# mokemokechicken/reversi-alpha-zero

Hardware: NVIDIA H100
Metric: self_play_games_per_sec (higher is better)
Workload: dtype f16

## Files before the change

### reversi-alpha-zero_b200/csrc/rz_net_tc.cu

```cuda
#include <stdlib.h>
#include <mutex>
#include <type_traits>
#include "rz_bitboard.cuh"
#include "rz_net.cuh"
#include "rz_tc_common.cuh"

namespace rz {
namespace tc {

constexpr int kThreads = 384;
constexpr uint32_t kProducerRegs = 40, kMathRegs = 232;
constexpr int kMathThreads = 256;
constexpr uint32_t kActCg = 2896, kActSlot = 144;
constexpr uint32_t kActBytes = 32 * kActCg;
constexpr uint32_t kStageBytes = 32768, kStages = 3;
constexpr int kResAhead = 4;
constexpr uint32_t kA0Bytes = 8192, kW0Bytes = 16384;
constexpr uint32_t kOffAct = 0;
constexpr uint32_t kOffW = kOffAct + kActBytes;
constexpr uint32_t kOffA0 = kOffW + kStages * kStageBytes;
constexpr uint32_t kOffW0 = kOffA0 + kA0Bytes;
constexpr uint32_t kOffSS = kOffW0 + kW0Bytes;
constexpr uint32_t kOffHw = kOffSS + 2 * 2048;
constexpr uint32_t kOffBar = kOffHw + 768 * 4;
constexpr uint32_t kNumBars = 2 * kStages + 1;
constexpr uint32_t kSmemBytes = kOffBar + kNumBars * 8;
constexpr uint32_t kSmemAlloc = kSmemBytes + 128;
static_assert(kSmemAlloc <= 232448, "shared memory budget exceeded");
static_assert(kTowerResFloatsPerCta == (size_t)kMathThreads * 128, "residual scratch per CTA");

#ifdef RZ_TOWER_STAMPS
enum : int {
    kStTiles,
    kStTile,
    kStKLoop,
    kStFull,
    kStMma,
    kStEpiBar,
    kStEpi0,
    kStEpi1,
    kStEpi2,
    kStEpiLast,
    kStFeat,
    kStEmpty,
    kStCount
};
constexpr int kStMaxCtas = 1024;
__device__ unsigned long long g_tower_stamps[kStMaxCtas][kStCount];
__device__ __forceinline__ void stamp_add(int phase, uint32_t cycles) { atomicAdd(&g_tower_stamps[blockIdx.x][phase], (unsigned long long)cycles); }
#define RZ_STAMP(...) __VA_ARGS__
#else
#define RZ_STAMP(...)
#endif

template <int CL>
__global__ void __launch_bounds__(kThreads, 1) net_tower_kernel(const Params pp) {
    Params p = pp;
    if (p.n_dev) p.n = *p.n_dev;
    extern __shared__ uint8_t smem_raw[];
    const uint32_t base = (smem_u32(smem_raw) + 127u) & ~127u;
    uint8_t* sm = smem_raw + (base - smem_u32(smem_raw));
    const int warp = threadIdx.x >> 5, lane = threadIdx.x & 31;
    const uint32_t bar0 = base + kOffBar;
    auto bar_full = [&](uint32_t s) { return bar0 + s * 8; };
    auto bar_empty = [&](uint32_t s) { return bar0 + (kStages + s) * 8; };
    const uint32_t bar_w0 = bar0 + 2 * kStages * 8;
    const uint32_t ntiles = (p.n + 1) >> 1;
    const int L = p.n_layers;
    const uint32_t crank = CL > 1 ? cluster_ctarank() : 0u;
    const uint32_t cbase = blockIdx.x - crank;
    const uint32_t iters = cbase < ntiles ? (ntiles - cbase + gridDim.x - 1) / gridDim.x : 0u;

    for (uint32_t i = threadIdx.x * 16; i < kActBytes; i += kThreads * 16) *reinterpret_cast<uint4*>(sm + kOffAct + i) = make_uint4(0, 0, 0, 0);
    fence_proxy_async();
    for (uint32_t i = threadIdx.x; i < 768; i += kThreads)
        reinterpret_cast<float*>(sm + kOffHw)[i] = __ldg(i < 512 ? p.blob + p.off_policy_conv + i : p.blob + p.off_value_conv + (i - 512));
    if (threadIdx.x == 0) {
        for (uint32_t s = 0; s < kStages; ++s) { mbar_init(bar_full(s), 1); mbar_init(bar_empty(s), 8 * CL); }
        mbar_init(bar_w0, 1);
        asm volatile("fence.mbarrier_init.release.cluster;" ::: "memory");
    }
    __syncthreads();
    if (CL > 1) cluster_sync_all();

    if (warp >= 8) {
        asm volatile("setmaxnreg.dec.sync.aligned.u32 %0;" ::"n"(kProducerRegs));
        if (warp == 8 && lane == 0) {
            if (iters > 0) {
                mbar_expect_tx(bar_w0, kW0Bytes);
                bulk_g2s(base + kOffW0, p.w0, kW0Bytes, bar_w0);
            }
            uint32_t stage = 0, phase = 0;
            for (uint32_t it = 0; it < iters; ++it) {
                for (int l = 1; l < L; ++l) {
                    const uint8_t* src = reinterpret_cast<const uint8_t*>(p.w) + (size_t)(l - 1) * 36 * kStageBytes;
                    RZ_STAMP(uint32_t st_empty = 0;)
                    for (int s = 0; s < 36; ++s) {
                        RZ_STAMP(const uint32_t c0 = (uint32_t)clock();)
                        mbar_wait(bar_empty(stage), phase ^ 1);
                        RZ_STAMP(st_empty += (uint32_t)clock() - c0;)
                        mbar_expect_tx(bar_full(stage), kStageBytes);
                        if (CL == 1) {
                            bulk_g2s(base + kOffW + stage * kStageBytes, src + (size_t)s * kStageBytes, kStageBytes, bar_full(stage));
                        } else {
                            constexpr uint32_t kSlice = kStageBytes / CL;
                            bulk_g2s_mc(base + kOffW + stage * kStageBytes + crank * kSlice, src + (size_t)s * kStageBytes + crank * kSlice,
                                        kSlice, bar_full(stage), (uint16_t)((1u << CL) - 1u));
                        }
                        if (++stage == kStages) { stage = 0; phase ^= 1; }
                    }
                    RZ_STAMP(stamp_add(kStEmpty, st_empty);)
                }
            }
        }
    } else {
        asm volatile("setmaxnreg.inc.sync.aligned.u32 %0;" ::"n"(kMathRegs));
        const int et = threadIdx.x;
        const int wg = warp >> 2;
        const int r0 = wg * 64 + (warp & 3) * 16 + (lane >> 2);
        const int g0 = r0 >> 3, x = r0 & 7, y = g0 >> 1;
        const int cq = 2 * (lane & 3);
        const uint32_t act_row0 = base + kOffAct + (g0 + 2) * kActSlot + (x + 1) * 16 + cq * 2;
        const uint32_t act_row1 = act_row0 + kActSlot;
        const uint32_t a_wg = base + kOffAct + wg * 8 * kActSlot;
        float* ss_s = reinterpret_cast<float*>(sm + kOffSS);
        float4* res = reinterpret_cast<float4*>(p.res + (size_t)blockIdx.x * kTowerResFloatsPerCta) + et;
        const float* hw = reinterpret_cast<const float*>(sm + kOffHw);
        uint32_t stage = 0, phase = 0, ss_buf = 0;
        float d[128];
        ss_s[et] = __ldg(p.ss + et);
        ss_s[256 + et] = __ldg(p.ss + 256 + et);

        for (uint32_t it = 0; it < iters; ++it) {
            const uint32_t tile = blockIdx.x + it * gridDim.x;
            const uint32_t pos0 = tile * 2;
            RZ_STAMP(const uint32_t st_tile0 = (uint32_t)clock();)
            {
                const int m = et & 127, g = m >> 3, brd = g & 1;
                const bool valid = pos0 + brd < p.n;
                build_layer0_operand(sm + kOffA0, valid ? p.own[pos0 + brd] : 0, valid ? p.enemy[pos0 + brd] : 0, 2 * (et >> 7), g, m & 7,
                                     g >> 1);
                fence_proxy_async();
            }
            float hs[6];
            for (int l = 0; l < L; ++l) {
                const float* sc = ss_s + ss_buf * 512;
                const bool is_conv2 = l > 0 && (l & 1) == 0;
                float4 rb[kResAhead];
                RZ_STAMP(uint32_t st_c = (uint32_t)clock(), st_bar = 0, st_full = 0, st_mma = 0;)
                epi_bar();
                RZ_STAMP(st_bar += (uint32_t)clock() - st_c;)
                {
                    const size_t nl = l + 1 < L ? (size_t)l + 1 : 0;
                    const uint32_t dst = smem_u32(ss_s + (ss_buf ^ 1) * 512 + et);
                    cp_async_4(dst, p.ss + nl * 512 + et);
                    cp_async_4(dst + 1024, p.ss + nl * 512 + 256 + et);
                }
                RZ_STAMP(const uint32_t st_k0 = (uint32_t)clock();)
                acc_fence(d);
                if (l == 0) {
                    RZ_STAMP(st_c = (uint32_t)clock();)
                    mbar_wait(bar_w0, 0);
                    RZ_STAMP(st_full += (uint32_t)clock() - st_c;)
                    wgmma_fence();
#pragma unroll
                    for (uint32_t j = 0; j < 2; ++j)
                        wgmma_m64n256k16(d, smem_desc(base + kOffA0 + j * 2 * 2048 + wg * 1024, 2048, 128),
                                         smem_desc(base + kOffW0 + j * 2 * 4096, 4096, 128), j);
                    wgmma_commit();
                    RZ_STAMP(st_c = (uint32_t)clock();)
                    wgmma_wait<0>();
                    RZ_STAMP(st_mma += (uint32_t)clock() - st_c;)
                } else {
                    int prev = -1;
                    for (uint32_t tap = 0; tap < 9; ++tap) {
                        const uint32_t a_tap = a_wg + (2 * (tap / 3)) * kActSlot + (tap % 3) * 16;
                        for (uint32_t kb = 0; kb < 4; ++kb) {
                            RZ_STAMP(st_c = (uint32_t)clock();)
                            mbar_wait(bar_full(stage), phase);
                            RZ_STAMP(st_full += (uint32_t)clock() - st_c;)
                            const uint32_t b_st = base + kOffW + stage * kStageBytes;
                            wgmma_fence();
#pragma unroll
                            for (uint32_t j = 0; j < 4; ++j)
                                wgmma_m64n256k16(d, smem_desc(a_tap + (kb * 8 + 2 * j) * kActCg, kActCg, kActSlot),
                                                 smem_desc(b_st + 2 * j * 4096, 4096, 128), (tap | kb | j) != 0);
                            wgmma_commit();
                            RZ_STAMP(st_c = (uint32_t)clock();)
                            wgmma_wait<1>();
                            RZ_STAMP(st_mma += (uint32_t)clock() - st_c;)
                            if (prev >= 0 && lane == 0) {
                                mbar_arrive(bar_empty(prev));
                                if (CL > 1) mbar_arrive_cta(bar_empty(prev), crank ^ 1u);
                            }
                            prev = (int)stage;
                            if (++stage == kStages) { stage = 0; phase ^= 1; }
                        }
                    }
                    if (is_conv2) {
#pragma unroll
                        for (int i = 0; i < kResAhead; ++i) rb[i] = res[i * 256];
                    }
                    RZ_STAMP(st_c = (uint32_t)clock();)
                    wgmma_wait<0>();
                    RZ_STAMP(st_mma += (uint32_t)clock() - st_c;)
                    if (lane == 0) {
                        mbar_arrive(bar_empty(prev));
                        if (CL > 1) mbar_arrive_cta(bar_empty(prev), crank ^ 1u);
                    }
                }
                RZ_STAMP(const uint32_t st_k1 = (uint32_t)clock();)
                acc_fence(d);
                cp_async_wait_all();
                ss_buf ^= 1;
                const bool keep_res = l == 0 || is_conv2;
                const bool last = l == L - 1;
                RZ_STAMP(st_c = (uint32_t)clock();)
                if (!last) epi_bar();
                RZ_STAMP(const uint32_t st_e0 = (uint32_t)clock(); st_bar += st_e0 - st_c;)
                float* dbg0 = nullptr;
                float* dbg1 = nullptr;
                if (last && p.dbg_tower) {
                    if (pos0 < p.n) dbg0 = p.dbg_tower + ((size_t)pos0 * 64 + y * 8 + x) * 256;
                    if (pos0 + 1 < p.n) dbg1 = p.dbg_tower + ((size_t)(pos0 + 1) * 64 + y * 8 + x) * 256;
                }
                constexpr int kEpiRelu = 0, kEpiKeep = 1, kEpiLast = 2;
                auto epilogue = [&](auto conv2, auto kind) {
                    constexpr bool kConv2 = decltype(conv2)::value;
                    constexpr bool kKeep = decltype(kind)::value == kEpiKeep, kLast = decltype(kind)::value == kEpiLast;
                    if (kLast) {
#pragma unroll
                        for (int k = 0; k < 6; ++k) hs[k] = 0.f;
                    }
#pragma unroll
                for (int i = 0; i < 32; ++i) {
                    const int c = 8 * i + cq;
                    const float2 s = *reinterpret_cast<const float2*>(sc + c);
                    const float2 b = *reinterpret_cast<const float2*>(sc + 256 + c);
                    float v0 = fmaf(d[4 * i + 0], s.x, b.x), v1 = fmaf(d[4 * i + 1], s.y, b.y);
                    float v2 = fmaf(d[4 * i + 2], s.x, b.x), v3 = fmaf(d[4 * i + 3], s.y, b.y);
                    if (kConv2) {
                        const float4 r = rb[i % kResAhead];
                        if (i + kResAhead < 32) rb[i % kResAhead] = res[(i + kResAhead) * 256];
                        v0 += r.x; v1 += r.y; v2 += r.z; v3 += r.w;
                    }
                    if (kKeep || kLast) {
                        v0 = fmaxf(v0, 0.f); v1 = fmaxf(v1, 0.f); v2 = fmaxf(v2, 0.f); v3 = fmaxf(v3, 0.f);
                    }
                    if (!kLast) {
                        if (kKeep) res[i * 256] = make_float4(v0, v1, v2, v3);
                        const uint32_t h0 = pack_h2<!kKeep>(v0, v1);
                        const uint32_t h1 = pack_h2<!kKeep>(v2, v3);
                        const uint32_t off = (c >> 3) * kActCg;
                        asm volatile("st.shared.b32 [%0], %1;" ::"r"(act_row0 + off), "r"(h0) : "memory");
                        asm volatile("st.shared.b32 [%0], %1;" ::"r"(act_row1 + off), "r"(h1) : "memory");
                    } else {
                        const float4 w = *reinterpret_cast<const float4*>(hw + 2 * c);
                        const float2 wv = *reinterpret_cast<const float2*>(hw + 512 + c);
                        hs[0] = fmaf(v1, w.z, fmaf(v0, w.x, hs[0]));
                        hs[1] = fmaf(v1, w.w, fmaf(v0, w.y, hs[1]));
                        hs[2] = fmaf(v1, wv.y, fmaf(v0, wv.x, hs[2]));
                        hs[3] = fmaf(v3, w.z, fmaf(v2, w.x, hs[3]));
                        hs[4] = fmaf(v3, w.w, fmaf(v2, w.y, hs[4]));
                        hs[5] = fmaf(v3, wv.y, fmaf(v2, wv.x, hs[5]));
                        if (dbg0) *reinterpret_cast<float2*>(dbg0 + c) = make_float2(v0, v1);
                        if (dbg1) *reinterpret_cast<float2*>(dbg1 + c) = make_float2(v2, v3);
                    }
                }
                };
                using Conv2 = std::true_type;
                using NoConv2 = std::false_type;
                if (last) {
                    if (is_conv2) epilogue(Conv2(), std::integral_constant<int, kEpiLast>());
                    else epilogue(NoConv2(), std::integral_constant<int, kEpiLast>());
                } else if (is_conv2) {
                    epilogue(Conv2(), std::integral_constant<int, kEpiKeep>());
                } else if (keep_res) {
                    epilogue(NoConv2(), std::integral_constant<int, kEpiKeep>());
                } else {
                    epilogue(NoConv2(), std::integral_constant<int, kEpiRelu>());
                }
                if (!last) fence_proxy_async();
                RZ_STAMP(if (et == 0) {
                    stamp_add(kStKLoop, st_k1 - st_k0); stamp_add(kStFull, st_full); stamp_add(kStMma, st_mma); stamp_add(kStEpiBar, st_bar);
                    stamp_add(l == 0 ? kStEpi0 : last ? kStEpiLast : is_conv2 ? kStEpi2 : kStEpi1, (uint32_t)clock() - st_e0);
                })
            }
            RZ_STAMP(const uint32_t st_h0 = (uint32_t)clock();)
#pragma unroll
            for (int k = 0; k < 6; ++k) {
                hs[k] += __shfl_xor_sync(0xffffffffu, hs[k], 1);
                hs[k] += __shfl_xor_sync(0xffffffffu, hs[k], 2);
            }
            {
                const int q = lane & 3;
                if (q < 2 && pos0 + q < p.n) {
                    const float h0 = q ? hs[3] : hs[0], h1 = q ? hs[4] : hs[1], h2 = q ? hs[5] : hs[2];
                    store_head_features(p.feat + (size_t)(pos0 + q) * kHeadFeatures, p.ss + (size_t)L * 512, y * 8 + x, h0 + 0.f,
                                        h1 + 0.f, h2 + 0.f);
                }
            }
            RZ_STAMP(if (et == 0) {
                const uint32_t st_h1 = (uint32_t)clock();
                stamp_add(kStFeat, st_h1 - st_h0); stamp_add(kStTile, st_h1 - st_tile0); stamp_add(kStTiles, 1);
            })
        }
    }

    __syncthreads();
    if (CL > 1) cluster_sync_all();
}

__global__ void pack_w0_kernel(const float* __restrict__ k0, __half* __restrict__ out) {
    const int i = blockIdx.x * blockDim.x + threadIdx.x;
    if (i >= 4 * 256 * 8) return;
    const int j = i & 7, n = (i >> 3) & 255, kc = i >> 11, k = kc * 8 + j;
    out[i] = __float2half_rn(k < 18 ? k0[(size_t)k * 256 + n] : 0.f);
}
__global__ void pack_w_kernel(const float* __restrict__ blob, size_t off_res0, size_t stride, int n_layers, __half* __restrict__ out) {
    const size_t total = (size_t)n_layers * 36 * 8 * 256 * 8;
    for (size_t i = (size_t)blockIdx.x * blockDim.x + threadIdx.x; i < total; i += (size_t)gridDim.x * blockDim.x) {
        const int j = i & 7, n = (i >> 3) & 255, kc = (i >> 11) & 7;
        const size_t ls = i >> 14;
        const int s = (int)(ls % 36), l = (int)(ls / 36);
        const int tap = s >> 2, kb = s & 3, ci = kb * 64 + kc * 8 + j;
        out[i] = __float2half_rn(blob[off_res0 + (size_t)l * stride + ((size_t)tap * 256 + ci) * 256 + n]);
    }
}

}

int net_pack_tc(rz_net* net, cudaStream_t stream) {
    tc::pack_w0_kernel<<<(4 * 256 * 8 + 255) / 256, 256, 0, stream>>>(net->blob + net->off_conv0, net->tc_w0);
    if (net->cfg.res_blocks > 0)
        tc::pack_w_kernel<<<num_sms() * 8, 256, 0, stream>>>(net->blob, net->off_res0, net->res_stride_conv, 2 * net->cfg.res_blocks, net->tc_w);
    RZ_LAUNCH_CHECK();
    return RZ_OK;
}

static int g_cluster = 0;

int set_tower_cluster(int cluster) {
    RZ_REQUIRE(cluster == 1 || cluster == 2, "rz_net_set_tower_cluster: cluster must be 1 or 2");
    g_cluster = cluster;
    return RZ_OK;
}

int tower_cluster() {
    if (g_cluster == 0) {
        const char* cs = getenv("RZ_TOWER_CLUSTER");
        g_cluster = (cs && atoi(cs) == 1) ? 1 : 2;
    }
    return g_cluster;
}

int net_forward_tc(rz_net* net, const uint64_t* own, const uint64_t* enemy, float* policy, float* value, size_t n, cudaStream_t stream,
                   float* dbg_tower, const uint32_t* n_dev, float* dbg_logits, float* dbg_vlogit) {
    if (net->cfg.filters == 64 || net->cfg.filters == 128)
        return net_forward_tc_narrow(net, own, enemy, policy, value, n, stream, dbg_tower, n_dev, dbg_logits, dbg_vlogit);
    RZ_REQUIRE(net->cfg.filters == 256, "wgmma tower requires 64, 128 or 256 filters (got %d)", net->cfg.filters);
    RZ_REQUIRE(net->cfg.value_fc <= (int)tc::kTcMaxV, "wgmma tower supports value_fc_size <= %u", tc::kTcMaxV);
    RZ_REQUIRE(n < (1ull << 31), "batch too large");
    static int max_pairs = -1;
    if (max_pairs < 0) {
        RZ_CUDA_TRY(cudaFuncSetAttribute(tc::net_tower_kernel<1>, cudaFuncAttributeMaxDynamicSharedMemorySize, (int)tc::kSmemAlloc));
        RZ_CUDA_TRY(cudaFuncSetAttribute(tc::net_tower_kernel<2>, cudaFuncAttributeMaxDynamicSharedMemorySize, (int)tc::kSmemAlloc));
        cudaLaunchConfig_t cfg = {};
        cfg.gridDim = dim3((unsigned)num_sms() & ~1u); cfg.blockDim = dim3(tc::kThreads); cfg.dynamicSmemBytes = tc::kSmemAlloc;
        cudaLaunchAttribute attr[1];
        attr[0].id = cudaLaunchAttributeClusterDimension;
        attr[0].val.clusterDim.x = 2; attr[0].val.clusterDim.y = 1; attr[0].val.clusterDim.z = 1;
        cfg.attrs = attr; cfg.numAttrs = 1;
        RZ_CUDA_TRY(cudaOccupancyMaxActiveClusters(&max_pairs, tc::net_tower_kernel<2>, &cfg));
    }
    const int cluster = tower_cluster() == 2 && max_pairs >= 1 ? 2 : 1;
    tc::Params p;
    p.w0 = net->tc_w0; p.w = net->tc_w; p.ss = net->scale_shift; p.blob = net->blob;
    p.off_policy_conv = net->off_policy_conv; p.off_policy_fc_k = net->off_policy_fc_k; p.off_policy_fc_b = net->off_policy_fc_b;
    p.off_value_conv = net->off_value_conv; p.off_value_fc1_k = net->off_value_fc1_k; p.off_value_fc1_b = net->off_value_fc1_b;
    p.off_value_fc2_k = net->off_value_fc2_k; p.off_value_fc2_b = net->off_value_fc2_b;
    p.own = own; p.enemy = enemy; p.policy = policy; p.value = value; p.dbg_tower = dbg_tower;
    p.dbg_logits = dbg_logits; p.dbg_vlogit = dbg_vlogit;
    p.n = (uint32_t)n; p.n_dev = n_dev; p.n_layers = 1 + 2 * net->cfg.res_blocks; p.V = net->cfg.value_fc;
    p.res = net->res;
    std::lock_guard<std::mutex> lock(tower_mutex());
    RZ_TRY(head_features(net, n));
    p.feat = net->feat;
    RZ_CUDA_TRY(cudaStreamWaitEvent(stream, net->res_done, 0));
    const uint32_t ntiles = (uint32_t)((n + 1) / 2);
    uint32_t grid = ntiles < (uint32_t)num_sms() ? ntiles : (uint32_t)num_sms();
    if (cluster == 1) {
        tc::net_tower_kernel<1><<<grid, tc::kThreads, tc::kSmemAlloc, stream>>>(p);
    } else {
        grid = (grid + 1) & ~1u;
        if (grid > 2u * (uint32_t)max_pairs) grid = 2u * (uint32_t)max_pairs;
        cudaLaunchConfig_t cfg = {};
        cfg.gridDim = dim3(grid); cfg.blockDim = dim3(tc::kThreads); cfg.dynamicSmemBytes = tc::kSmemAlloc; cfg.stream = stream;
        cudaLaunchAttribute attr[1];
        attr[0].id = cudaLaunchAttributeClusterDimension;
        attr[0].val.clusterDim.x = 2; attr[0].val.clusterDim.y = 1; attr[0].val.clusterDim.z = 1;
        cfg.attrs = attr; cfg.numAttrs = 1;
        RZ_CUDA_TRY(cudaLaunchKernelEx(&cfg, tc::net_tower_kernel<2>, p));
    }
    RZ_LAUNCH_CHECK();
    RZ_TRY(net_heads(p, stream));
    RZ_CUDA_TRY(cudaEventRecord(net->res_done, stream));
    return RZ_OK;
}

}

#ifdef RZ_TOWER_STAMPS
extern "C" int rz_tower_stamps(unsigned long long* out, int n_ctas, int reset) {
    using namespace rz::tc;
    if (n_ctas < 0 || n_ctas > kStMaxCtas) return (int)cudaErrorInvalidValue;
    const size_t bytes = (size_t)n_ctas * kStCount * sizeof(unsigned long long);
    cudaError_t e = cudaDeviceSynchronize();
    if (e == cudaSuccess && out) e = cudaMemcpyFromSymbol(out, g_tower_stamps, bytes);
    if (e == cudaSuccess && reset) {
        void* dev = nullptr;
        e = cudaGetSymbolAddress(&dev, g_tower_stamps);
        if (e == cudaSuccess) e = cudaMemset(dev, 0, sizeof(g_tower_stamps));
        if (e == cudaSuccess) e = cudaDeviceSynchronize();
    }
    return (int)e;
}
extern "C" int rz_tower_stamp_count() { return rz::tc::kStCount; }
#endif
```

### reversi-alpha-zero_b200/csrc/rz_tc_common.cuh

```cuda
#pragma once
#include <cuda_fp16.h>
#include "rz_bitboard.cuh"
#include "rz_net.cuh"

namespace rz {
namespace tc {

__device__ __forceinline__ uint32_t smem_u32(const void* p) { return (uint32_t)__cvta_generic_to_shared(p); }

__device__ __forceinline__ void mbar_init(uint32_t bar, uint32_t count) {
    asm volatile("mbarrier.init.shared::cta.b64 [%0], %1;" ::"r"(bar), "r"(count) : "memory");
}
__device__ __forceinline__ void mbar_expect_tx(uint32_t bar, uint32_t bytes) {
    asm volatile("mbarrier.arrive.expect_tx.shared::cta.b64 _, [%0], %1;" ::"r"(bar), "r"(bytes) : "memory");
}
__device__ __forceinline__ void mbar_arrive(uint32_t bar) {
    asm volatile("mbarrier.arrive.shared::cta.b64 _, [%0];" ::"r"(bar) : "memory");
}
__device__ __forceinline__ void mbar_arrive_cta(uint32_t bar, uint32_t rank) {
    uint32_t remote;
    asm volatile("mapa.shared::cluster.u32 %0, %1, %2;" : "=r"(remote) : "r"(bar), "r"(rank));
    asm volatile("mbarrier.arrive.shared::cluster.b64 _, [%0];" ::"r"(remote) : "memory");
}
__device__ __forceinline__ void mbar_wait(uint32_t bar, uint32_t parity) {
    uint32_t ok = 0;
    long long t0 = 0;
    for (uint32_t spin = 0; !ok; ++spin) {
        asm volatile(
            "{\n\t.reg .pred p;\n\t"
            "mbarrier.try_wait.parity.shared::cta.b64 p, [%1], %2;\n\t"
            "selp.u32 %0, 1, 0, p;\n\t}"
            : "=r"(ok)
            : "r"(bar), "r"(parity)
            : "memory");
        if (!ok && (spin & 1023) == 1023) {
            const long long now = clock64();
            if (t0 == 0) t0 = now;
            else if (now - t0 > 8000000000LL) __trap();
        }
    }
}
__device__ __forceinline__ void bulk_g2s(uint32_t dst, const void* src, uint32_t bytes, uint32_t bar) {
    asm volatile("cp.async.bulk.shared::cluster.global.mbarrier::complete_tx::bytes [%0], [%1], %2, [%3];" ::"r"(dst), "l"(src),
                 "r"(bytes), "r"(bar)
                 : "memory");
}
__device__ __forceinline__ void bulk_g2s_mc(uint32_t dst, const void* src, uint32_t bytes, uint32_t bar, uint16_t mask) {
    asm volatile(
        "cp.async.bulk.shared::cluster.global.mbarrier::complete_tx::bytes.multicast::cluster [%0], [%1], %2, [%3], %4;" ::"r"(dst),
        "l"(src), "r"(bytes), "r"(bar), "h"(mask)
        : "memory");
}
__device__ __forceinline__ void cluster_sync_all() {
    asm volatile("barrier.cluster.arrive.release.aligned;\n\tbarrier.cluster.wait.acquire.aligned;" ::: "memory");
}
__device__ __forceinline__ uint32_t cluster_ctarank() {
    uint32_t r;
    asm volatile("mov.u32 %0, %%cluster_ctarank;" : "=r"(r));
    return r;
}
__device__ __forceinline__ void cp_async_4(uint32_t dst, const void* src) {
    asm volatile("cp.async.ca.shared.global [%0], [%1], 4;" ::"r"(dst), "l"(src) : "memory");
}
__device__ __forceinline__ void cp_async_wait_all() { asm volatile("cp.async.wait_all;" ::: "memory"); }
__device__ __forceinline__ void fence_proxy_async() { asm volatile("fence.proxy.async.shared::cta;" ::: "memory"); }
__device__ __forceinline__ void epi_bar() { asm volatile("bar.sync 1, 256;" ::: "memory"); }

__device__ __forceinline__ uint64_t smem_desc(uint32_t addr, uint32_t lbo, uint32_t sbo) {
    return (uint64_t)((addr >> 4) & 0x3FFF) | ((uint64_t)((lbo >> 4) & 0x3FFF) << 16) | ((uint64_t)((sbo >> 4) & 0x3FFF) << 32);
}
__device__ __forceinline__ void wgmma_fence() { asm volatile("wgmma.fence.sync.aligned;" ::: "memory"); }
__device__ __forceinline__ void wgmma_commit() { asm volatile("wgmma.commit_group.sync.aligned;" ::: "memory"); }
template <int N>
__device__ __forceinline__ void wgmma_wait() { asm volatile("wgmma.wait_group.sync.aligned %0;" ::"n"(N) : "memory"); }
__device__ __forceinline__ void acc_fence(float (&d)[128]) {
#pragma unroll
    for (int i = 0; i < 128; ++i) asm volatile("" : "+f"(d[i])::"memory");
}

#define RZ_D4(i) "+f"(d[i]), "+f"(d[i + 1]), "+f"(d[i + 2]), "+f"(d[i + 3])
#define RZ_D16(i) RZ_D4(i), RZ_D4(i + 4), RZ_D4(i + 8), RZ_D4(i + 12)
__device__ __forceinline__ void wgmma_m64n256k16(float (&d)[128], uint64_t adesc, uint64_t bdesc, uint32_t accumulate) {
    asm volatile(
        "{\n\t.reg .pred p;\n\t"
        "setp.ne.b32 p, %130, 0;\n\t"
        "wgmma.mma_async.sync.aligned.m64n256k16.f32.f16.f16 {"
        "%0, %1, %2, %3, %4, %5, %6, %7, %8, %9, %10, %11, %12, %13, %14, %15, "
        "%16, %17, %18, %19, %20, %21, %22, %23, %24, %25, %26, %27, %28, %29, %30, %31, "
        "%32, %33, %34, %35, %36, %37, %38, %39, %40, %41, %42, %43, %44, %45, %46, %47, "
        "%48, %49, %50, %51, %52, %53, %54, %55, %56, %57, %58, %59, %60, %61, %62, %63, "
        "%64, %65, %66, %67, %68, %69, %70, %71, %72, %73, %74, %75, %76, %77, %78, %79, "
        "%80, %81, %82, %83, %84, %85, %86, %87, %88, %89, %90, %91, %92, %93, %94, %95, "
        "%96, %97, %98, %99, %100, %101, %102, %103, %104, %105, %106, %107, %108, %109, %110, %111, "
        "%112, %113, %114, %115, %116, %117, %118, %119, %120, %121, %122, %123, %124, %125, %126, %127"
        "}, %128, %129, p, 1, 1, 0, 0;\n\t}"
        : RZ_D16(0), RZ_D16(16), RZ_D16(32), RZ_D16(48), RZ_D16(64), RZ_D16(80), RZ_D16(96), RZ_D16(112)
        : "l"(adesc), "l"(bdesc), "r"(accumulate)
        : "memory");
}
template <int O>
__device__ __forceinline__ void wgmma_m64n128k16(float (&d)[128], uint64_t adesc, uint64_t bdesc, uint32_t accumulate) {
    asm volatile(
        "{\n\t.reg .pred p;\n\t"
        "setp.ne.b32 p, %66, 0;\n\t"
        "wgmma.mma_async.sync.aligned.m64n128k16.f32.f16.f16 {"
        "%0, %1, %2, %3, %4, %5, %6, %7, %8, %9, %10, %11, %12, %13, %14, %15, "
        "%16, %17, %18, %19, %20, %21, %22, %23, %24, %25, %26, %27, %28, %29, %30, %31, "
        "%32, %33, %34, %35, %36, %37, %38, %39, %40, %41, %42, %43, %44, %45, %46, %47, "
        "%48, %49, %50, %51, %52, %53, %54, %55, %56, %57, %58, %59, %60, %61, %62, %63"
        "}, %64, %65, p, 1, 1, 0, 0;\n\t}"
        : RZ_D16(O), RZ_D16(O + 16), RZ_D16(O + 32), RZ_D16(O + 48)
        : "l"(adesc), "l"(bdesc), "r"(accumulate)
        : "memory");
}
template <int O>
__device__ __forceinline__ void wgmma_m64n64k16(float (&d)[128], uint64_t adesc, uint64_t bdesc, uint32_t accumulate) {
    asm volatile(
        "{\n\t.reg .pred p;\n\t"
        "setp.ne.b32 p, %34, 0;\n\t"
        "wgmma.mma_async.sync.aligned.m64n64k16.f32.f16.f16 {"
        "%0, %1, %2, %3, %4, %5, %6, %7, %8, %9, %10, %11, %12, %13, %14, %15, "
        "%16, %17, %18, %19, %20, %21, %22, %23, %24, %25, %26, %27, %28, %29, %30, %31"
        "}, %32, %33, p, 1, 1, 0, 0;\n\t}"
        : RZ_D16(O), RZ_D16(O + 16)
        : "l"(adesc), "l"(bdesc), "r"(accumulate)
        : "memory");
}
#undef RZ_D16
#undef RZ_D4

template <bool RELU>
__device__ __forceinline__ uint32_t pack_h2(float a, float b) {
    uint32_t d;
    if (RELU) asm("cvt.rn.relu.satfinite.f16x2.f32 %0, %1, %2;" : "=r"(d) : "f"(b), "f"(a));
    else      asm("cvt.rn.satfinite.f16x2.f32 %0, %1, %2;" : "=r"(d) : "f"(b), "f"(a));
    return d;
}

struct Params {
    const __half* w0;
    const __half* w;
    const float* ss;
    const float* blob;
    size_t off_policy_conv, off_policy_fc_k, off_policy_fc_b, off_value_conv, off_value_fc1_k, off_value_fc1_b, off_value_fc2_k,
        off_value_fc2_b;
    const u64* own;
    const u64* enemy;
    float* policy;
    float* value;
    float* res;
    float* feat;
    float* dbg_tower;
    float* dbg_logits;
    float* dbg_vlogit;
    uint32_t n;
    const uint32_t* n_dev;
    int n_layers;
    int V;
};

constexpr uint32_t kTcMaxV = 512;

__device__ __forceinline__ void build_layer0_operand(uint8_t* a0, u64 o, u64 e, int kc0, int g, int x, int y) {
#pragma unroll
    for (int kk = 0; kk < 2; ++kk) {
        const int kc = kc0 + kk;
        uint32_t w[4];
#pragma unroll
        for (int jp = 0; jp < 4; ++jp) {
            uint32_t packed = 0;
#pragma unroll
            for (int half = 0; half < 2; ++half) {
                const int k = kc * 8 + jp * 2 + half;
                uint32_t bit = 0;
                if (k < 18) {
                    const int tap = k >> 1, yy = y + tap / 3 - 1, xx = x + tap % 3 - 1;
                    if (yy >= 0 && yy < 8 && xx >= 0 && xx < 8) bit = (uint32_t)((((k & 1) ? e : o) >> (yy * 8 + xx)) & 1ULL);
                }
                packed |= (bit ? 0x3C00u : 0u) << (16 * half);
            }
            w[jp] = packed;
        }
        *reinterpret_cast<uint4*>(a0 + kc * 2048 + g * 128 + x * 16) = make_uint4(w[0], w[1], w[2], w[3]);
    }
}

__device__ __forceinline__ void store_head_features(float* f, const float* ssh, int pix, float a0, float a1, float av) {
    f[pix] = fmaxf(fmaf(a0, ssh[0], ssh[2]), 0.f);
    f[64 + pix] = fmaxf(fmaf(a1, ssh[1], ssh[3]), 0.f);
    f[128 + pix] = fmaxf(fmaf(av, ssh[4], ssh[5]), 0.f);
}

}

int net_heads(const tc::Params& p, cudaStream_t stream);

}
```

Baseline: 24.52.

## Interleave scale/bias in smem and store epilogue activations via stmatrix

The per-layer scale and bias arrays are now interleaved in shared memory, so each epilogue step fetches both with a single float4 load, prefetched a couple of iterations ahead. Activation stores switch from paired 32-bit st.shared per channel group to stmatrix.m8n8.x4, which writes two channel groups at once through a per-lane address computed for the stmatrix fragment layout. This cuts the number of shared-memory store and load instructions in the tower epilogue. The cost is extra live registers and a new address mapping that has to match the existing activation layout exactly.

```diff
diff --git a/reversi-alpha-zero_b200/csrc/rz_net_tc.cu b/reversi-alpha-zero_b200/csrc/rz_net_tc.cu
--- a/reversi-alpha-zero_b200/csrc/rz_net_tc.cu
+++ b/reversi-alpha-zero_b200/csrc/rz_net_tc.cu
@@ -15,6 +15,7 @@
 constexpr uint32_t kActBytes = 32 * kActCg;
 constexpr uint32_t kStageBytes = 32768, kStages = 3;
 constexpr int kResAhead = 4;
+constexpr int kSsAhead = 2;
 constexpr uint32_t kA0Bytes = 8192, kW0Bytes = 16384;
 constexpr uint32_t kOffAct = 0;
 constexpr uint32_t kOffW = kOffAct + kActBytes;
@@ -120,16 +121,16 @@
         const int r0 = wg * 64 + (warp & 3) * 16 + (lane >> 2);
         const int g0 = r0 >> 3, x = r0 & 7, y = g0 >> 1;
         const int cq = 2 * (lane & 3);
-        const uint32_t act_row0 = base + kOffAct + (g0 + 2) * kActSlot + (x + 1) * 16 + cq * 2;
-        const uint32_t act_row1 = act_row0 + kActSlot;
+        const uint32_t act_st = base + kOffAct + (g0 + 2 + ((lane >> 3) & 1)) * kActSlot + ((lane & 7) + 1) * 16 + (lane >> 4) * kActCg;
         const uint32_t a_wg = base + kOffAct + wg * 8 * kActSlot;
         float* ss_s = reinterpret_cast<float*>(sm + kOffSS);
+        const int ss_i = (et & ~1) * 2 + (et & 1);
         float4* res = reinterpret_cast<float4*>(p.res + (size_t)blockIdx.x * kTowerResFloatsPerCta) + et;
         const float* hw = reinterpret_cast<const float*>(sm + kOffHw);
         uint32_t stage = 0, phase = 0, ss_buf = 0;
         float d[128];
-        ss_s[et] = __ldg(p.ss + et);
-        ss_s[256 + et] = __ldg(p.ss + 256 + et);
+        ss_s[ss_i] = __ldg(p.ss + et);
+        ss_s[ss_i + 2] = __ldg(p.ss + 256 + et);
 
         for (uint32_t it = 0; it < iters; ++it) {
             const uint32_t tile = blockIdx.x + it * gridDim.x;
@@ -152,9 +153,9 @@
                 RZ_STAMP(st_bar += (uint32_t)clock() - st_c;)
                 {
                     const size_t nl = l + 1 < L ? (size_t)l + 1 : 0;
-                    const uint32_t dst = smem_u32(ss_s + (ss_buf ^ 1) * 512 + et);
+                    const uint32_t dst = smem_u32(ss_s + (ss_buf ^ 1) * 512 + ss_i);
                     cp_async_4(dst, p.ss + nl * 512 + et);
-                    cp_async_4(dst + 1024, p.ss + nl * 512 + 256 + et);
+                    cp_async_4(dst + 8, p.ss + nl * 512 + 256 + et);
                 }
                 RZ_STAMP(const uint32_t st_k0 = (uint32_t)clock();)
                 acc_fence(d);
@@ -232,13 +233,17 @@
 #pragma unroll
                         for (int k = 0; k < 6; ++k) hs[k] = 0.f;
                     }
+                    uint32_t he0 = 0, he1 = 0;
+                    float4 sbr[kSsAhead];
+#pragma unroll
+                    for (int i = 0; i < kSsAhead; ++i) sbr[i] = *reinterpret_cast<const float4*>(sc + 2 * (8 * i + cq));
 #pragma unroll
                 for (int i = 0; i < 32; ++i) {
                     const int c = 8 * i + cq;
-                    const float2 s = *reinterpret_cast<const float2*>(sc + c);
-                    const float2 b = *reinterpret_cast<const float2*>(sc + 256 + c);
-                    float v0 = fmaf(d[4 * i + 0], s.x, b.x), v1 = fmaf(d[4 * i + 1], s.y, b.y);
-                    float v2 = fmaf(d[4 * i + 2], s.x, b.x), v3 = fmaf(d[4 * i + 3], s.y, b.y);
+                    const float4 sb = sbr[i % kSsAhead];
+                    if (i + kSsAhead < 32) sbr[i % kSsAhead] = *reinterpret_cast<const float4*>(sc + 2 * (c + 8 * kSsAhead));
+                    float v0 = fmaf(d[4 * i + 0], sb.x, sb.z), v1 = fmaf(d[4 * i + 1], sb.y, sb.w);
+                    float v2 = fmaf(d[4 * i + 2], sb.x, sb.z), v3 = fmaf(d[4 * i + 3], sb.y, sb.w);
                     if (kConv2) {
                         const float4 r = rb[i % kResAhead];
                         if (i + kResAhead < 32) rb[i % kResAhead] = res[(i + kResAhead) * 256];
@@ -251,9 +256,8 @@
                         if (kKeep) res[i * 256] = make_float4(v0, v1, v2, v3);
                         const uint32_t h0 = pack_h2<!kKeep>(v0, v1);
                         const uint32_t h1 = pack_h2<!kKeep>(v2, v3);
-                        const uint32_t off = (c >> 3) * kActCg;
-                        asm volatile("st.shared.b32 [%0], %1;" ::"r"(act_row0 + off), "r"(h0) : "memory");
-                        asm volatile("st.shared.b32 [%0], %1;" ::"r"(act_row1 + off), "r"(h1) : "memory");
+                        if (i & 1) stmatrix_x4(act_st + (i - 1) * kActCg, he0, he1, h0, h1);
+                        else { he0 = h0; he1 = h1; }
                     } else {
                         const float4 w = *reinterpret_cast<const float4*>(hw + 2 * c);
                         const float2 wv = *reinterpret_cast<const float2*>(hw + 512 + c);
diff --git a/reversi-alpha-zero_b200/csrc/rz_tc_common.cuh b/reversi-alpha-zero_b200/csrc/rz_tc_common.cuh
--- a/reversi-alpha-zero_b200/csrc/rz_tc_common.cuh
+++ b/reversi-alpha-zero_b200/csrc/rz_tc_common.cuh
@@ -63,6 +63,10 @@
     asm volatile("cp.async.ca.shared.global [%0], [%1], 4;" ::"r"(dst), "l"(src) : "memory");
 }
 __device__ __forceinline__ void cp_async_wait_all() { asm volatile("cp.async.wait_all;" ::: "memory"); }
+__device__ __forceinline__ void stmatrix_x4(uint32_t addr, uint32_t r0, uint32_t r1, uint32_t r2, uint32_t r3) {
+    asm volatile("stmatrix.sync.aligned.m8n8.x4.shared.b16 [%0], {%1, %2, %3, %4};" ::"r"(addr), "r"(r0), "r"(r1), "r"(r2), "r"(r3)
+                 : "memory");
+}
 __device__ __forceinline__ void fence_proxy_async() { asm volatile("fence.proxy.async.shared::cta;" ::: "memory"); }
 __device__ __forceinline__ void epi_bar() { asm volatile("bar.sync 1, 256;" ::: "memory"); }
 
```

Result: no change. 24.58, median of 6 (+0.2%).
